# Chthi/Ofighters

Hardware: AMD Instinct MI355X
Metric: arena-steps/sec (env.step+obs+policy fwd) at 4096 arenas, 1/2/4/8 MI355X (higher is better)
Workload: dtype f32; 1 GPU; 4096 arenas x 8 ships per GPU, random-bot actions + step + 2D obs rasterise (u8 maps) + bi-head policy forward for 8 ship(s)/arena, trunk shared per arena (BASELINE configs[3]); arenas_per_gpu=4096, ships=8, laser_cap=512, episode_ticks=200, parallelism=arena-sharded x1, RCCL all-reduce of episodic scores only, laser_overflow=0, last_episode_score_sum=70993, last_episode_arenas=4096

## Files before the change

include/ofx.h:

```cpp
#ifndef OFX_H
#define OFX_H

#include <stddef.h>
#include <stdint.h>

#ifdef __cplusplus
extern "C" {
#endif

#define OFX_VERSION 1

enum {
  OFX_OK = 0,
  OFX_ERR_INVALID = -1,
  OFX_ERR_NO_DEVICE = -2,
  OFX_ERR_HIP = -3,
  OFX_ERR_STATE = -4,
  OFX_ERR_OVERFLOW = -5
};

typedef struct ofx_config {
  int32_t n_arenas;
  int32_t n_ships;
  int32_t laser_cap;
// ... 141 lines not shown
  int32_t n_tensors;
} ofx_policy_desc;
int ofx_policy_layout(const ofx_handle *h, ofx_policy_desc *desc_host);
int ofx_policy_forward(ofx_handle *h, const float *weights, const uint8_t *ship_mask,
                       float *act_values, int32_t *iaction, int32_t *ipointer,
                       float *heatmap);
int ofx_policy_pin_weights(ofx_handle *h, const float *weights);
#define OFX_OPT_TRUNK_PLAIN 1
#define OFX_OPT_FRAMES_REF  2
#define OFX_OPT_TRUNK_FUSE  4
#define OFX_OPT_BILINEAR_LEGACY 3
#define OFX_OPT_POLICY_BF16 5
#define OFX_OPT_FIT_PLAIN 6
#define OFX_OPT_TRUNK_SPARSE 7
int ofx_policy_trunk_stats(ofx_handle *h, int64_t *counts_host);
int ofx_set_option(ofx_handle *h, int32_t option, int32_t value);
int ofx_policy_explore(ofx_handle *h, double epsilon, uint64_t seed, uint32_t tick, int32_t collecting,
                       const uint8_t *ship_mask, int32_t *iaction, int32_t *ipointer);
int ofx_policy_epsilon_ladder(ofx_handle *h, const double *expo_host);
int ofx_policy_epsilon_ladder_host(ofx_handle *h, double *dst_host);
int ofx_policy_act(ofx_handle *h, const float *weights, const uint8_t *ship_mask, double epsilon, uint64_t seed,
                   uint32_t tick, int32_t collecting, float *q_sa, float *p_sp, float *v_act, float *v_ptr);
int ofx_policy_act_boltzmann(ofx_handle *h, const float *weights, const uint8_t *ship_mask, double epsilon,
                             float tau_act, float tau_ptr, uint64_t seed, uint32_t tick, int32_t collecting,
                             float *q_sa, float *p_sp, float *v_act, float *v_ptr);
int ofx_policy_gumbel(ofx_handle *h, const uint32_t *words_dev, int32_t n, float *g_dev);
int ofx_policy_actions(ofx_handle *h, const int32_t *iaction, const int32_t *ipointer,
                       const uint8_t *ship_mask, ofx_action *actions);

typedef struct ofx_transition {
// ... 125 lines not shown
```

ofighters_amd/_native.py:

```python
import ctypes as C
import os

_HERE = os.path.dirname(os.path.abspath(__file__))
LIB_PATH = os.path.join(_HERE, "libofx.so")

OFX_OK = 0
OFX_ERR_INVALID = -1
OFX_ERR_NO_DEVICE = -2
OFX_ERR_HIP = -3
OFX_ERR_STATE = -4
OFX_ERR_OVERFLOW = -5

BOT_IDLE, BOT_RANDOM, BOT_TURRET, BOT_RUNNER, BOT_THRUST, BOT_SHOOT = range(6)
BEHAVIOURS = {None: BOT_IDLE, "idle": BOT_IDLE, "random": BOT_RANDOM, "turret": BOT_TURRET,
              "runner": BOT_RUNNER, "thrust": BOT_THRUST, "shoot": BOT_SHOOT}

(F_SHIP_X, F_SHIP_Y, F_SHIP_PX, F_SHIP_PY, F_SHIP_ALIVE, F_REWARD, F_SCORE, F_N_LASERS, F_LASER_X, F_LASER_Y,
 F_LASER_OWNER, F_LASER_DEAD, F_KILLER, F_TIME, F_LAST_SCORES, F_HULL, F_LASER_DX, F_LASER_DY,
 F_OBS_REWARD) = range(19)

MAP_U8, MAP_F32, MAP_F64, MAP_BITS = range(4)
OPT_TRUNK_PLAIN, OPT_FRAMES_REF, OPT_BILINEAR_LEGACY, OPT_TRUNK_FUSE, OPT_POLICY_BF16, OPT_FIT_PLAIN, OPT_TRUNK_SPARSE = 1, 2, 3, 4, 5, 6, 7


# ... 140 lines not shown
    "ofx_dqn_targets_nstep": (_i, [_vp, _vp, C.c_int32, _vp, _vp, _vp, _vp, _vp, _vp, _vp, _vp, _vp]),
    "ofx_dqn_targets_double": (_i, [_vp, _vp, _vp, C.c_int32, _vp, _vp, _vp, C.c_float, _vp, _vp, _vp, _vp, _vp, _vp]),
    "ofx_policy_blend_weights": (_i, [_vp, _vp, _vp, C.c_float]),
    "ofx_policy_forward_obs_soft": (_i, [_vp, _vp, C.c_int32, _vp, _vp, C.c_float, _vp, _vp, _vp, _vp, _vp, _vp, _vp, _vp, _vp]),
    "ofx_dqn_targets_soft": (_i, [_vp, _vp, C.c_int32, _vp, _vp, _vp, C.c_float, _vp, _vp, C.c_float, C.c_float, C.c_float,
                                  C.c_float, _vp, _vp, _vp, _vp]),
    "ofx_obs_transform": (_i, [_vp, C.c_int32, _vp, _vp, _vp, _vp]),
    "ofx_replay_augment": (_i, [_vp, _u64, _u32, C.c_int32, C.c_int32, _u32, _vp, _vp, _vp, _vp]),
    "ofx_timer_start": (_i, [_vp]),
    "ofx_timer_stop": (_i, [_vp, C.POINTER(C.c_float)]),
    "ofx_event_record": (_i, [_vp, C.c_int32]),
    "ofx_policy_profile": (_i, [_vp, C.c_int32]),
    "ofx_policy_pin_weights": (_i, [_vp, _vp]),
    "ofx_set_option": (_i, [_vp, C.c_int32, C.c_int32]),
    "ofx_policy_trunk_stats": (_i, [_vp, C.POINTER(C.c_int64)]),
    "ofx_event_elapsed": (_i, [_vp, C.c_int32, C.c_int32, C.POINTER(C.c_float)]),
}

_LIB = None


def lib():
    global _LIB
    if _LIB is None:
        if not os.path.exists(LIB_PATH):
            raise ImportError(
                "ofighters_amd: %s is missing - build it with `make -C ofighters_amd/csrc` "
                "(there is no CPU fallback)" % LIB_PATH)
        L = C.CDLL(LIB_PATH)
        for name, (res, args) in SIGNATURES.items():
# ... 21 lines not shown
```

ofighters_amd/csrc/ofx_policy.hip:

```cpp
#include <string.h>

#include "ofx_internal.h"
#include "ofx_arena.h"
#include "ofx_blob.h"
#include "ofx_trunk.h"
#include "ofx_head.h"

typedef float f32x16 __attribute__((ext_vector_type(16)));
typedef float f32x4 __attribute__((ext_vector_type(4)));


extern "C" int ofx_policy_layout(const ofx_handle *h, ofx_policy_desc *desc) {
  (void)h;
  if (!desc) { ofx_set_error("ofx_policy_layout: null desc"); return OFX_ERR_INVALID; }
  memset(desc, 0, sizeof(*desc));
  desc->n_tensors = policy_layout(desc->offset, desc->count);
  desc->n_floats = desc->offset[desc->n_tensors];
  return OFX_OK;
}

struct PrepLayout {
  int tw[4], tb[4];
  int uw[3], ub[3];
  int w3mf;
// ... 574 lines not shown
  const int a = s / M, i = s - a * M;
  const float a0 = act[2 * s], a1 = act[2 * s + 1], T = t_act[s];
  int ia = a1 > a0 ? 1 : 0;
  if (T != 0.f) {
    uint32_t r[4];
    ofx_philox4x32_10((uint32_t)(arena_base + a), (uint32_t)i, tick, OFX_STREAM_BOLTZMANN_ACT, k0, k1, r);
    ia = fmaf(T, hd_gumbel(r[1]), a1) > fmaf(T, hd_gumbel(r[0]), a0) ? 1 : 0;
  }
  iaction[s] = ia;
  q_sa[s] = ia ? a1 : a0;
  v_act[s] = fmaxf(a0, a1);
}

struct PolicyWs {
  float *p1, *p2, *p3, *p4, *g1, *d1, *u0, *up1, *u2fr, *vfr, *c4;
  unsigned long long *best;
  int32_t *iaction, *ipointer, *live;
  float *t_act, *t_ptr, *cand_raw;
  unsigned long long *cand_key;
  unsigned *cand_max;
  float *soft_m, *soft_z;
};

constexpr int kDense1Chunks = 25;

static void policy_layout_ws(Arena &A, bool fused, size_t N, size_t S, bool sample, bool soft, PolicyWs &W) {
  size_t f2, f3, f4;
  ofx_head_frame_bytes(S, &f2, &f3, &f4);
  W.p1 = A.f(fused ? 0 : N * 8 * 200 * 200);
  W.p2 = A.f(N * 8 * 100 * 100); W.p3 = A.f(N * 8 * 50 * 50); W.p4 = A.f(N * 5000); W.g1 = A.f(N * 100 * kDense1Chunks);
  W.d1 = A.f(S * 100); W.u0 = A.f(S * 625); W.up1 = A.f(S * 2 * 50 * 50);
  W.u2fr = (float *)A.take(f2); W.vfr = (float *)A.take(f3); W.c4 = (float *)A.take(f4);
  W.best = A.n<unsigned long long>(S); W.iaction = A.n<int32_t>(S); W.ipointer = A.n<int32_t>(2 * S); W.live = A.n<int32_t>(S + 1);
  const size_t Q = sample ? S : 0;
  W.t_act = A.f(Q); W.t_ptr = A.f(Q); W.cand_raw = A.f(8 * Q); W.cand_key = A.n<unsigned long long>(8 * Q); W.cand_max = A.n<unsigned>(8 * Q);
  const size_t Qs = soft ? S : 0;
  W.soft_m = A.f(8 * Qs); W.soft_z = A.f(8 * Qs);
}
static int policy_workspace(ofx_handle *h, PolicyWs *ws, size_t N, size_t S, bool sample = false, bool soft = false) {
  const bool fused = ofx_trunk_fused(h, N);
  Arena measure;
  policy_layout_ws(measure, fused, N, S, sample, soft, *ws);
  const int rc = ofx_ensure_scratch(h, measure.used);
  if (rc) return rc;
  Arena A(h->scratch, measure.used);
  policy_layout_ws(A, fused, N, S, sample, soft, *ws);
  if (!A.ok()) { ofx_set_error("policy forward: internal workspace sized too small"); return OFX_ERR_STATE; }
  return OFX_OK;
}

int ofx_launch_gemm(ofx_handle *h, const float *A, int lda, const float *B, int ldb, const float *bias, float *C, int ldc,
                    int M, int N, int K, int relu, const int32_t *live) {
  const int tiles_m = (M + 31) / 32, tiles_n = (N + 31) / 32, tiles = tiles_m * tiles_n;
  if (K == 100 && lda % 4 == 0 && ((uintptr_t)A & 15) == 0)
    hipLaunchKernelGGL(k_gemm_f32_k100, dim3((unsigned)(((tiles_m + 3) / 4) * tiles_n)), dim3(256), 0, h->stream, A, lda, B, ldb,
                       bias, C, ldc, M, N, relu, live, tiles_n);
  else
    hipLaunchKernelGGL(k_gemm_f32, dim3((tiles + 3) / 4), dim3(256), 0, h->stream, A, lda, B, ldb, bias, C, ldc, M, N, K,
                       relu, live);
  OFX_HIP(hipGetLastError());
  return OFX_OK;
}

// ... 43 lines not shown
  if (h->prep_pinned && h->prep_pinned == weights) return policy_prepare(h, weights, &h->prep);
  return OFX_OK;
}

extern "C" int ofx_set_option(ofx_handle *h, int32_t option, int32_t value) {
  if (!h) { ofx_set_error("ofx_set_option: null handle"); return OFX_ERR_INVALID; }
  switch (option) {
    case OFX_OPT_TRUNK_PLAIN: h->opt_trunk_plain = value != 0; return OFX_OK;
    case OFX_OPT_TRUNK_FUSE:
      if (value < 0 || value > 2) { ofx_set_error("ofx_set_option: OFX_OPT_TRUNK_FUSE takes 0 (auto), 1 (always), 2 (never)"); return OFX_ERR_INVALID; }
      h->opt_trunk_fuse = value; return OFX_OK;
    case OFX_OPT_FRAMES_REF: h->opt_frames_ref = value != 0; return OFX_OK;
    case OFX_OPT_TRUNK_SPARSE:
      if (value && !h->trunk_stat) {
        OFX_HIP(hipSetDevice(h->cfg.device));
        OFX_HIP(hipMalloc((void **)&h->trunk_stat, 4 * sizeof(unsigned long long)));
        OFX_HIP(hipMemsetAsync(h->trunk_stat, 0, 4 * sizeof(unsigned long long), h->stream));
      }
      h->opt_trunk_dense = value == 0; h->opt_trunk_count = value != 0; return OFX_OK;
    case OFX_OPT_FIT_PLAIN: h->opt_fit_plain = value != 0; return OFX_OK;
    case OFX_OPT_POLICY_BF16:
      if (value < 0 || value > 2) { ofx_set_error("ofx_set_option: OFX_OPT_POLICY_BF16 takes 0 (fp32), 1 (bf16 operands), 2 (fp16 operands)"); return OFX_ERR_INVALID; }
      h->opt_policy_lowp = value; return OFX_OK;
    case OFX_OPT_BILINEAR_LEGACY:
      if (h->opt_bilinear_legacy == (value != 0)) return OFX_OK;
      h->opt_bilinear_legacy = value != 0;
      OFX_HIP(hipSetDevice(h->cfg.device));
      return h->prep_pinned ? policy_prepare(h, h->prep_pinned, &h->prep) : OFX_OK;
    default: ofx_set_error("ofx_set_option: unknown option %d", option); return OFX_ERR_INVALID;
  }
}

// ... 24 lines not shown
  int32_t off[64], cnt[64];
  policy_layout(off, cnt);
  const PrepLayout L = prep_layout();

  const bool pinned = h->prep && h->prep_pinned == weights;
  if (!pinned && (rc = policy_prepare(h, weights, &h->prep_tmp))) return rc;
  const float *prep = pinned ? h->prep : h->prep_tmp;

  const int lowp = a.vec8 == nullptr ? h->opt_policy_lowp : 0;
  TrunkParams tp;
  memset(&tp, 0, sizeof(tp));
  tp.bits[0] = a.bits[0]; tp.bits[1] = a.bits[1]; tp.bits_stride = a.bits_stride; tp.images = N;
  for (int i = 0; i < 4; i++) { tp.tw[i] = prep + L.tw[i]; tp.tb[i] = prep + L.tb[i]; }
  for (int i = 0; i < 3; i++) tp.wbm[i] = prep + L.wbm[i];
  tp.lut1 = prep + L.lut1; tp.zero16 = prep + L.zero16;
  tp.p1 = ws.p1; tp.p2 = ws.p2; tp.p3 = ws.p3; tp.p4 = ws.p4;
  tp.lowp = lowp; tp.sparse = !h->opt_trunk_dense || a.vec8 != nullptr;
  tp.stat = h->opt_trunk_count ? h->trunk_stat : nullptr;
  if ((rc = ofx_launch_trunk(h, tp))) return rc;

  const float *k1 = weights + off[OFX_T_DENSE1];
  {
    static_assert(5000 == kDense1Chunks * kSplitKc, "k_gemm_f32_splitk's chunk");
    const int tiles_n = (100 + 31) / 32, groups_m = ((N + 31) / 32 + 3) / 4;
    hipLaunchKernelGGL(k_gemm_f32_splitk, dim3((unsigned)(tiles_n * groups_m * kDense1Chunks)), dim3(256), 0, h->stream, ws.p4,
                       5000, k1 + 8 * 100, 100, ws.g1, N, 100, tiles_n, groups_m);
    OFX_HIP(hipGetLastError());
  }
  HeadParams hp;
  hp.N = N; hp.M = a.M; hp.st = h->st; hp.vec8 = a.vec8; hp.g1 = ws.g1; hp.g1_chunks = kDense1Chunks;
  hp.k1 = k1; hp.b1 = weights + off[OFX_T_DENSE1 + 1];
// ... 380 lines not shown
```

ofighters_amd/csrc/ofx_trunk.h:

```cpp
#pragma once
#include "ofx_internal.h"

#define PS 400

struct ConvParams {
  const float *in;
  const unsigned *bits[2];
  size_t bits_stride;
  const float *w, *b;
  float *out;
  const uint8_t *mask;
  const float *wbm;
  int H, W;
  int tiles_x, tiles;
  int legacy;
  int images;
  const int32_t *live;
  unsigned long long *stat;
};

struct TrunkParams {
  const unsigned *bits[2];
  size_t bits_stride;
  int images;
  const float *tw[4], *tb[4], *wbm[3], *lut1, *zero16;
  float *p1, *p2, *p3, *p4;
  int lowp;
  bool sparse;
  unsigned long long *stat;
};

bool ofx_trunk_fused(const ofx_handle *h, size_t images);
int ofx_launch_trunk(ofx_handle *h, const TrunkParams &p);
int ofx_launch_conv1_lut(ofx_handle *h, const void *bits, int n, const float *lut, float *out);
```

ofighters_amd/csrc/ofx_trunk.hip:

```cpp
#include "ofx_trunk.h"
#include "ofx_diag.h"
#include "ofx_lowp.h"

typedef float f32x4 __attribute__((ext_vector_type(4)));
typedef float f32x2 __attribute__((ext_vector_type(2)));

template <int CIN, int COUT, int TH, int TW, int MODE, bool POOL, bool OUT_HWC>
__global__ __launch_bounds__(((TH / 2) * (TW / 2) + 63) / 64 * 64) void k_conv(ConvParams p) {
  constexpr int NT = (TH / 2) * (TW / 2);
  constexpr int NTB = (NT + 63) / 64 * 64;
  constexpr int TWP = TW + 2;
  __shared__ __align__(16) float tile[CIN][TH + 2][TWP];
  const int img = blockIdx.x / p.tiles, t = blockIdx.x - img * p.tiles;
  if (p.mask && !p.mask[img]) return;
  const int ty0 = (t / p.tiles_x) * TH, tx0 = (t % p.tiles_x) * TW;
  const int tid = threadIdx.x;
  const int H = p.H, W = p.W;

  constexpr int TOTAL = CIN * (TH + 2) * TWP;
  constexpr int SU = 8;
  for (int base = 0; base < TOTAL; base += NTB * SU) {
    float vals[SU];
#pragma unroll
    for (int u = 0; u < SU; u++) {
// ... 409 lines not shown
      } else {
        f32x4 d0 = binit;
#pragma unroll
        for (int j = 0; j < NK; j++) d0 = __builtin_amdgcn_mfma_f32_16x16x4f32(a0[aof(j)], bw[j], d0, 0, 0, 0);
        finish(d0, T);
      }
    }
  }
}

template <int WD, int RP, int LS, int PLS, int LP>
__device__ __forceinline__ void ts_gemm_phase_sparse(const float *abase, const float (&bw)[LP ? 1 : 24], const lp_x4 (&bwb)[6],
                                                     const f32x4 binit, int wv, int lane,
                                                     int n16, int kq, int r, float *orow, const unsigned *nz, float k2,
                                                     bool top, bool bottom, unsigned &n_exec, unsigned &n_all,
                                                     unsigned long long *dbg = nullptr) {
#if OFX_TRUNK_STAMPS
  unsigned long long g_last = __builtin_amdgcn_s_memtime();
#define TSG_STAMP(i) do { const unsigned long long t_ = __builtin_amdgcn_s_memtime(); dbg[i] += t_ - g_last; g_last = t_; } while (0)
#else
#define TSG_STAMP(i) do { } while (0)
#endif
  constexpr int NK = 24, NPX = RP * WD, NT = (NPX + 15) / 16;
  static_assert(WD % 4 == 0 && NT <= 64, "four M-tiles per wave at most");
  auto aof = [&](int j) -> int { return (4 * (j & 1)) * PLS + ((j >> 1) / 3) * LS + ((j >> 1) % 3); };
  int toff[6];
#pragma unroll
  for (int J = 0; J < 6; J++) {
    const int tap = 2 * J + (kq >> 1);
    toff[J] = (4 * (kq & 1) - kq) * PLS + (tap / 3) * LS + tap % 3;
  }
// ... 31 lines not shown
    float q0, q1;
    q0 = max_raw(max_raw(d[0], 0.f), d[1]);
    q1 = max_raw(max_raw(d[2], 0.f), d[3]);
    q0 = max_raw(q0, __builtin_bit_cast(float, __builtin_amdgcn_mov_dpp(__builtin_bit_cast(int, q0), 0xB1, 0xF, 0xF, true)));
    q1 = max_raw(q1, __builtin_bit_cast(float, __builtin_amdgcn_mov_dpp(__builtin_bit_cast(int, q1), 0xB1, 0xF, 0xF, true)));
    const int P = 16 * T + 4 * kq;
    const int rp = P / WD, x = P - rp * WD;
    if (r == 0 && P < NPX) *reinterpret_cast<float2 *>(orow + rp * (WD / 2) + (x >> 1)) = make_float2(q0, q1);
  };
  auto a_of_tile = [&](int T) -> const float * {
    const int P = min(16 * T + n16, NPX - 1);
    const int rp = P / WD, x = P - rp * WD;
    return abase + 2 * rp * LS + x;
  };
  unsigned long long run_mask;
  {
    const int T = lane, P = 16 * T, rp = P / WD, x = P - rp * WD;
    bool run = T < NT;
    if (run && !(x < 1 || x + 15 > WD - 2 || P + 15 >= NPX || (top && rp == 0) || (bottom && rp == RP - 1))) {
      const int w0 = (x - 1) >> 5, lo = (x - 1) & 31;
      const unsigned m0 = 0x3FFFFu << lo, m1 = lo + 18 > 32 ? (1u << (lo + 18 - 32)) - 1u : 0u;
      unsigned any = 0u;
#pragma unroll
      for (int rr = 0; rr < 4; rr++) {
        const unsigned *rw = nz + (2 * rp + rr) * 8 + w0;
        any |= (rw[0] & m0) | (rw[1] & m1);
      }
      run = any != 0u;
    }
    run_mask = __builtin_amdgcn_ballot_w64(run);
  }
  auto store_const = [&](int T) {
    const int P = 16 * T + 4 * kq, rp = P / WD, x = P - rp * WD;
    if (r == 0) *reinterpret_cast<float2 *>(orow + rp * (WD / 2) + (x >> 1)) = make_float2(k2, k2);
  };
  auto run1 = [&](int T0) {
    f32x4 d0 = binit;
    mm1(a_of_tile(T0), d0);
    finish(d0, T0);
  };
#pragma unroll 1
  for (int T = wv; T < NT; T += 16)
    if (!((run_mask >> T) & 1ull)) store_const(T);
  if (wv == 0) { n_all += (unsigned)NT; n_exec += (unsigned)__builtin_popcountll(run_mask); }
  TSG_STAMP(0);
  unsigned long long m = run_mask;
  for (int i = 0; i < wv && m; i++) m &= m - 1;
#pragma unroll 1
  while (m) {
    const int T0 = __builtin_ctzll(m);
    unsigned long long m2 = m;
    for (int i = 0; i < 16 && m2; i++) m2 &= m2 - 1;
    if (m2) {
      const int T1 = __builtin_ctzll(m2);
      f32x4 d0 = binit, d1 = binit;
      mm2(a_of_tile(T0), a_of_tile(T1), d0, d1);
      finish(d0, T0);
      finish(d1, T1);
      for (int i = 0; i < 16 && m2; i++) m2 &= m2 - 1;
    } else run1(T0);
    m = m2;
  }
  TSG_STAMP(2);
}

template <int WD, int RP, int LS, int PLS, int LP>
__device__ __forceinline__ void ts_gemm_phase_bf16(const float *abase, const lp_x4 (&bwb)[6], const f32x4 binit, int wv, int n16,
                                                   int kq, int r, float *orow) {
  constexpr int NPX = RP * WD, NT = (NPX + 15) / 16;
  static_assert(WD % 4 == 0 && NT <= 64, "four M-tiles per wave at most");
  int toff[6];
#pragma unroll
  for (int J = 0; J < 6; J++) {
    const int tap = 2 * J + (kq >> 1);
    toff[J] = (4 * (kq & 1) - kq) * PLS + (tap / 3) * LS + tap % 3;
  }
// ... 23 lines not shown
      const float *q0 = a0 + toff[J], *q1 = a1 + toff[J];
      const lp_x4 A0 = lp_pk4<LP>(q0[0], q0[PLS], q0[2 * PLS], q0[3 * PLS]);
      const lp_x4 A1 = lp_pk4<LP>(q1[0], q1[PLS], q1[2 * PLS], q1[3 * PLS]);
      d0 = lp_mfma16<LP>(A0, bwb[J], d0);
      d1 = lp_mfma16<LP>(A1, bwb[J], d1);
    }
    finish(d0, T);
    if (two) finish(d1, T1);
  }
}

constexpr int F12_TH = 10, F12_LS = 216, F12_ROWS = F12_TH + 2;
constexpr int F12_PLS = (F12_ROWS * F12_LS + 63) / 64 * 64 + 16;
constexpr int F12_WR = 14, F12_BR = 2 * (F12_TH + 1) + 2;
constexpr int F12_THREADS = 1024;
static_assert(F12_PLS % 64 == 16 && F12_PLS % 4 == 0 && F12_LS % 4 == 0, "tile layout");
static_assert(2 * F12_BR * F12_WR <= F12_THREADS, "one staged word per thread");
static_assert((F12_TH + 1) * 100 <= 2 * F12_THREADS && F12_TH * 100 <= F12_THREADS, "pixel pairs per step");

template <int LP, bool SPARSE = false>
__global__ __launch_bounds__(F12_THREADS) void k_trunk12(ConvParams p, const float *lut) {
  constexpr bool BF16 = LP != 0;
  constexpr int W = PS, H = PS, H1 = PS / 2, H2 = PS / 4, LS = F12_LS, PLS = F12_PLS, NK = 24;
  __shared__ __align__(16) float slut[2 * 512 * 8];
  __shared__ __align__(16) float tile[8 * F12_PLS];
  __shared__ unsigned rows[2][2][F12_BR][F12_WR];
  __shared__ __align__(16) float halo[2][8][2][F12_LS];
  __shared__ unsigned nz[SPARSE ? 2 : 1][F12_ROWS][8];
  __shared__ __align__(16) float k1s[8], k2s[8];
  __shared__ float wbs[(SPARSE && !BF16) ? 24 * 64 : 1];
  unsigned n_exec = 0, n_all = 0, t_exec = 0, t_all = 0;
#if OFX_TRUNK_STAMPS
  unsigned long long st_a = 0, st_b = 0, st_last = __builtin_amdgcn_s_memtime(), st_begin = st_last, st_g[3] = {0, 0, 0};
#define T12_STAMP(acc) do { const unsigned long long t_ = __builtin_amdgcn_s_memtime(); acc += t_ - st_last; st_last = t_; } while (0)
#else
#define T12_STAMP(acc) do { } while (0)
#endif
  const int tid = threadIdx.x, lane = tid & 63;
  const int wv = __builtin_amdgcn_readfirstlane(tid >> 6);
  const int n16 = lane & 15, kq = lane >> 4, co = n16 >> 1, r = n16 & 1;

  auto bits_fetch = [&](int img, int pa, int pb) -> unsigned {
    const int nrows = 2 * (pb - pa) + 2;
    unsigned out = 0u;
// ... 51 lines not shown
      f32x4 d0 = binit;
      if constexpr (BF16) {
#pragma unroll
        for (int J = 0; J < 6; J++) {
          const int tap = 2 * J + (kq >> 1);
          const float *q0 = a0 + (4 * (kq & 1) - kq) * PLS + (tap / 3) * LS + tap % 3;
          d0 = lp_mfma16<LP ? LP : 1>(lp_pk4<LP ? LP : 1>(q0[0], q0[PLS], q0[2 * PLS], q0[3 * PLS]), bwb[J], d0);
        }
      } else {
        auto aof = [&](int j) -> int { return (4 * (j & 1)) * PLS + ((j >> 1) / 3) * LS + ((j >> 1) % 3); };
#pragma unroll
        for (int j = 0; j < NK; j++) d0 = __builtin_amdgcn_mfma_f32_16x16x4f32(a0[aof(j)], wbs[(BF16 ? 0 : j) * 64 + lane], d0, 0, 0, 0);
      }
      float q0 = max_raw(max_raw(d0[0], 0.f), d0[1]);
      q0 = max_raw(q0, __builtin_bit_cast(float, __builtin_amdgcn_mov_dpp(__builtin_bit_cast(int, q0), 0xB1, 0xF, 0xF, true)));
      if (r == 0 && kq == 0) k2s[co] = q0;
    }
    __syncthreads();
    for (int e = tid; e < 8 * PLS / 4; e += F12_THREADS) reinterpret_cast<f32x4 *>(tile)[e] = f32x4{0.f, 0.f, 0.f, 0.f};
  }
  bits_commit(0, 0, F12_TH + 1, bits_fetch((int)blockIdx.x, 0, F12_TH + 1));
  unsigned w_ahead = 0u;
  if constexpr (SPARSE) { if ((int)blockIdx.x < p.images) w_ahead = bits_fetch((int)blockIdx.x, F12_TH + 1, 2 * F12_TH + 1); }
  __syncthreads();
  const float k2 = SPARSE ? k2s[co] : 0.f;

#pragma unroll 1
  for (int img = (int)blockIdx.x; img < p.images; img += (int)gridDim.x)
#pragma unroll 1
  for (int step = 0; step < H1 / F12_TH; step++) {
    const int R0 = step * F12_TH;
// ... 85 lines not shown
      if (++s2 == H1 / F12_TH) { s2 = 0; i2 += (int)gridDim.x; }
      const int r2 = s2 * F12_TH;
      w_ahead = i2 < p.images ? bits_fetch(i2, s2 ? r2 + 1 : 0, min(r2 + F12_TH + 1, H1)) : 0u;
    }

    if constexpr (SPARSE) {
      float bwl[BF16 ? 1 : NK];
      if constexpr (!BF16) {
        int zoff;
        asm volatile("s_mov_b32 %0, 0" : "=s"(zoff));
#pragma unroll
        for (int j = 0; j < NK; j++) bwl[j] = wbs[j * 64 + lane + zoff];
      }
      ts_gemm_phase_sparse<200, F12_TH / 2, F12_LS, F12_PLS, LP>(abase, bwl, bwb, binit, wv, lane, n16, kq, r,
                                                                  p.out + (((size_t)img * 8 + co) * H2 + (R0 >> 1)) * H2,
                                                                  &nz[buf][0][0], k2, step == 0, last, n_exec, n_all
#if OFX_TRUNK_STAMPS
                                                                  , st_g
#endif
                                                                  );
      for (int e = tid; e < F12_ROWS * 8; e += F12_THREADS) (&nz[buf ^ 1][0][0])[e] = 0u;
    } else if constexpr (BF16)
      ts_gemm_phase_bf16<200, F12_TH / 2, F12_LS, F12_PLS, LP ? LP : 1>(abase, bwb, binit, wv, n16, kq, r,
                                                            p.out + (((size_t)img * 8 + co) * H2 + (R0 >> 1)) * H2);
    else
      ts_gemm_phase<200, F12_TH / 2, F12_LS, F12_PLS>(abase, bw, binit, wv, n16, kq, r,
                                                       p.out + (((size_t)img * 8 + co) * H2 + (R0 >> 1)) * H2);
    if constexpr (!SPARSE) { if (more) bits_commit(buf ^ 1, na, nb, nextw); }
    __syncthreads();
  }
  if constexpr (SPARSE) {
#if OFX_TRUNK_STAMPS
    T12_STAMP(st_b);
    if (p.stat && tid == 0) {
      atomicAdd(&p.stat[0], st_a); atomicAdd(&p.stat[1], st_b);
      atomicAdd(&p.stat[2], st_g[0]); atomicAdd(&p.stat[3], st_g[2]);
    }
#else
    if (p.stat && lane == 0) {
      atomicAdd(&p.stat[0], (unsigned long long)n_exec); atomicAdd(&p.stat[1], (unsigned long long)n_all);
      atomicAdd(&p.stat[2], (unsigned long long)t_exec); atomicAdd(&p.stat[3], (unsigned long long)t_all);
    }
#endif
  }
}

constexpr int C3_W = 100, C3_TH = 20, C3_LS = 108, C3_ROWS = C3_TH + 2, C3_F4 = C3_LS / 4;
constexpr int C3_PLS = (C3_ROWS * C3_LS + 63) / 64 * 64 + 16;
constexpr int C3_PF4 = C3_ROWS * C3_F4, C3_NI = (C3_PF4 + 63) / 64;
static_assert(C3_PLS % 64 == 16 && C3_W % C3_TH == 0 && C3_W / 4 + 2 == C3_F4 && 64 * C3_NI * 4 <= C3_PLS + 64 * 4, "tile layout");
static_assert(2 * 8 * C3_PLS * 4 <= 160 * 1024, "two tiles in LDS");

template <int LP>
__global__ __launch_bounds__(F12_THREADS) void k_conv3_stream(ConvParams p, const float *zero16) {
  constexpr bool BF16 = LP != 0;
  constexpr int W = C3_W, H = C3_W, H2 = C3_W / 2, PLS = C3_PLS, NK = 24, STEPS = H / C3_TH;
  __shared__ __align__(16) float tiles[2][8 * C3_PLS];
  const int tid = threadIdx.x, lane = tid & 63;
  const int wv = __builtin_amdgcn_readfirstlane(tid >> 6);
  const int n16 = lane & 15, kq = lane >> 4, co = n16 >> 1, r = n16 & 1;

  auto stage = [&](int buf, int img, int R0) {
#pragma unroll 1
    for (int i = wv; i < 8 * C3_NI; i += F12_THREADS / 64) {
      const int ci = i / C3_NI, k = i - ci * C3_NI;
      const int q = 64 * k + lane;
      if (q < C3_PF4) {
        const int row = q / C3_F4, c4 = q - row * C3_F4, gy = R0 - 1 + row;
        const float *src = zero16;
        if (c4 >= 1 && c4 <= W / 4 && gy >= 0 && gy < H) src = p.in + (((size_t)img * 8 + ci) * H + gy) * W + 4 * (c4 - 1);
        __builtin_amdgcn_global_load_lds((const __attribute__((address_space(1))) void *)src,
                                         (__attribute__((address_space(3))) void *)&tiles[buf][ci * PLS + 256 * k], 16, 0, 0);
      }
    }
  };

  float bw[BF16 ? 1 : NK];
  lp_x4 bwb[6];
  if constexpr (BF16) ts_bw_lp<LP ? LP : 1>(p.wbm, n16, kq, bwb);
  else {
#pragma unroll
    for (int j = 0; j < NK; j++) bw[j] = p.wbm[j * 64 + lane];
  }
  const float bias = p.b[co];
  const f32x4 binit = {bias, bias, bias, bias};
  if ((int)blockIdx.x < p.images) stage(0, (int)blockIdx.x, 0);
  __builtin_amdgcn_s_waitcnt(0x0F70);
  __syncthreads();
  int buf = 0;
#pragma unroll 1
  for (int img = (int)blockIdx.x; img < p.images; img += (int)gridDim.x)
#pragma unroll 1
  for (int step = 0; step < STEPS; step++) {
    const int R0 = step * C3_TH;
    const bool last = step + 1 == STEPS;
    const int nimg = last ? img + (int)gridDim.x : img;
    if (nimg < p.images) stage(buf ^ 1, nimg, last ? 0 : R0 + C3_TH);
    if constexpr (BF16)
      ts_gemm_phase_bf16<W, C3_TH / 2, C3_LS, C3_PLS, LP ? LP : 1>(&tiles[buf][kq * PLS + 3], bwb, binit, wv, n16, kq, r,
                                                      p.out + (((size_t)img * 8 + co) * H2 + (R0 >> 1)) * H2);
    else
      ts_gemm_phase<W, C3_TH / 2, C3_LS, C3_PLS>(&tiles[buf][kq * PLS + 3], bw, binit, wv, n16, kq, r,
                                                 p.out + (((size_t)img * 8 + co) * H2 + (R0 >> 1)) * H2);
    __builtin_amdgcn_s_waitcnt(0x0F70);
    __syncthreads();
    buf ^= 1;
  }
}

bool ofx_trunk_fused(const ofx_handle *h, size_t N) {
  if (h->opt_trunk_plain) return false;
  return h->opt_trunk_fuse == 1 || (h->opt_trunk_fuse == 0 && N >= 4 * (size_t)h->n_cus);
}

template <int CIN, int COUT, int TH, int TW, int MODE, bool POOL, bool OUT_HWC>
static int launch_conv(ofx_handle *h, ConvParams p, int images, int H) {
  p.H = H; p.W = H;
  p.tiles_x = H / TW;
  p.tiles = p.tiles_x * (H / TH);
  constexpr int NTB = ((TH / 2) * (TW / 2) + 63) / 64 * 64;
  hipLaunchKernelGGL((k_conv<CIN, COUT, TH, TW, MODE, POOL, OUT_HWC>), dim3((unsigned)(images * p.tiles)), dim3(NTB), 0,
// ... 15 lines not shown
  cp.bits[1] = cp.bits[0] + (PS * PS) / 32;
  cp.bits_stride = 2 * (size_t)((PS * PS) / 32);
  cp.out = out; cp.images = n;
  return launch_conv1_lut(h, cp, lut);
}

static void trunk_layer(ConvParams &cp, const TrunkParams &p, int i, const float *in, float *out) {
  cp.in = in; cp.w = p.tw[i]; cp.b = p.tb[i]; cp.out = out;
  if (i > 0) cp.wbm = p.wbm[i - 1];
}

template <int LP>
static int trunk_streaming(ofx_handle *h, ConvParams cp, const TrunkParams &p) {
  const dim3 grid((unsigned)(p.images < h->n_cus ? p.images : h->n_cus));
  cp.w = p.tw[0]; cp.b = p.tb[1]; cp.out = p.p2; cp.wbm = p.wbm[0]; cp.stat = p.stat;
  if (p.sparse) hipLaunchKernelGGL((k_trunk12<LP, true>), grid, dim3(F12_THREADS), 0, h->stream, cp, p.lut1);
  else hipLaunchKernelGGL((k_trunk12<LP, false>), grid, dim3(F12_THREADS), 0, h->stream, cp, p.lut1);
  OFX_HIP(hipGetLastError());
  trunk_layer(cp, p, 2, p.p2, p.p3);
  hipLaunchKernelGGL(k_conv3_stream<LP>, grid, dim3(F12_THREADS), 0, h->stream, cp, p.zero16);
  OFX_HIP(hipGetLastError());
  trunk_layer(cp, p, 3, p.p3, p.p4);
  return launch_convm<8, 10, 4, 0, true, 1, LP>(h, cp, p.images, 50);
}

int ofx_launch_trunk(ofx_handle *h, const TrunkParams &p) {
  ConvParams cp{};
  cp.bits[0] = p.bits[0]; cp.bits[1] = p.bits[1]; cp.bits_stride = p.bits_stride; cp.images = p.images;
  const bool plain = h->opt_trunk_plain;
  if (ofx_trunk_fused(h, (size_t)p.images))
    return p.lowp == 1 ? trunk_streaming<1>(h, cp, p) : p.lowp == 2 ? trunk_streaming<2>(h, cp, p) : trunk_streaming<0>(h, cp, p);
  const int N = p.images;
  int rc;
  trunk_layer(cp, p, 0, nullptr, p.p1);
  if ((rc = plain ? launch_conv<2, 8, 10, 100, 1, true, false>(h, cp, N, 400) : launch_conv1_lut(h, cp, p.lut1))) return rc;
// ... 3 lines not shown
  if ((rc = plain ? launch_conv<8, 8, 10, 100, 0, true, false>(h, cp, N, 100) : launch_convm<8, 4, 7, 0, false, 1>(h, cp, N, 100))) return rc;
  trunk_layer(cp, p, 3, p.p3, p.p4);
  return plain ? launch_conv<8, 8, 10, 50, 0, true, true>(h, cp, N, 50) : launch_convm<8, 10, 4, 0, true, 1>(h, cp, N, 50);
}

extern "C" int ofx_policy_trunk_stats(ofx_handle *h, int64_t *counts_host) {
  if (!h || !counts_host) { ofx_set_error("ofx_policy_trunk_stats: null argument"); return OFX_ERR_INVALID; }
  for (int i = 0; i < 4; i++) counts_host[i] = 0;
  if (!h->trunk_stat) return OFX_OK;
  OFX_HIP(hipSetDevice(h->cfg.device));
  OFX_HIP(hipMemcpyAsync(counts_host, h->trunk_stat, 4 * sizeof(unsigned long long), hipMemcpyDeviceToHost, h->stream));
  OFX_HIP(hipMemsetAsync(h->trunk_stat, 0, 4 * sizeof(unsigned long long), h->stream));
  OFX_HIP(hipStreamSynchronize(h->stream));
  return OFX_OK;
}
```

ofighters_amd/engine.py:

```python
import ctypes as C

import numpy as np

from . import _native as nat

_FIELD_DTYPE = {
    nat.F_SHIP_X: np.int32, nat.F_SHIP_Y: np.int32, nat.F_SHIP_PX: np.int32, nat.F_SHIP_PY: np.int32,
    nat.F_SHIP_ALIVE: np.uint8, nat.F_REWARD: np.int32, nat.F_SCORE: np.int32, nat.F_N_LASERS: np.int32,
    nat.F_LASER_X: np.float64, nat.F_LASER_Y: np.float64, nat.F_LASER_OWNER: np.uint8,
    nat.F_LASER_DEAD: np.uint8, nat.F_KILLER: np.int16, nat.F_TIME: np.int32, nat.F_LAST_SCORES: np.int32,
    nat.F_HULL: np.int32, nat.F_LASER_DX: np.float64, nat.F_LASER_DY: np.float64, nat.F_OBS_REWARD: np.int32,
}
_MAP_DTYPE = {nat.MAP_U8: np.uint8, nat.MAP_F32: np.float32, nat.MAP_F64: np.float64, nat.MAP_BITS: np.uint8}

ACTION_DTYPE = np.dtype([("px", np.int32), ("py", np.int32), ("shoot", np.uint8), ("thrust", np.uint8),
                         ("valid", np.uint8), ("_pad", np.uint8)])
assert ACTION_DTYPE.itemsize == C.sizeof(nat.OfxAction) == 12


class DeviceBuffer:

    def __init__(self, nbytes):
        self.nbytes = int(nbytes)
        p = C.c_void_p()
# ... 322 lines not shown
                       heat_ptr=None):
        nat.check(nat.lib().ofx_policy_forward(self._h, weights_ptr, ship_mask_ptr, act_ptr, iaction_ptr,
                                               ipointer_ptr, heat_ptr))

    def policy_pin_weights(self, weights_ptr):
        nat.check(nat.lib().ofx_policy_pin_weights(self._h, weights_ptr))

    def set_option(self, option, value):
        nat.check(nat.lib().ofx_set_option(self._h, int(option), int(value)))

    def policy_trunk_stats(self):
        v = (C.c_int64 * 4)()
        nat.check(nat.lib().ofx_policy_trunk_stats(self._h, v))
        return tuple(int(x) for x in v)

    def policy_actions(self, out_ptr=None, iaction_ptr=None, ipointer_ptr=None, ship_mask_ptr=None):
        out_ptr = out_ptr or self._actions.ptr
        nat.check(nat.lib().ofx_policy_actions(self._h, iaction_ptr, ipointer_ptr, ship_mask_ptr, out_ptr))
        return out_ptr

    def policy_forward_host(self, weights, ship_mask=None, want_heat=False):
        S = self.N * self.M
        w = np.ascontiguousarray(weights, np.float32)
        dw = DeviceBuffer(w.nbytes).upload(w)
        dm = None
        if ship_mask is not None:
            m = np.ascontiguousarray(ship_mask, np.uint8).reshape(S)
            dm = DeviceBuffer(m.nbytes).upload(m)
        da, di, dp = DeviceBuffer(8 * S), DeviceBuffer(4 * S), DeviceBuffer(8 * S)
        dh = DeviceBuffer(4 * S * self.W * self.H) if want_heat else None
# ... 455 lines not shown
```

Measured before the change: 230,600 arena-steps/s.

## Propagate conv2 sparsity marks to skip constant tiles in streaming conv3

The fused conv1/2 kernel now writes per-row bitmasks of non-constant pooled outputs, plus the constant fill value K2, to global buffers. A new sparse variant of the streaming conv3 kernel loads these marks into LDS, precomputes the constant output K3, and runs only the MFMA tiles whose inputs are non-constant. The tile-distribution loop across waves is also replaced with a mbcnt/ballot rank, removing serial bit-popping. This adds mark stores and loads and a small one-time K3 computation per block, plus stats and debug entry points.

New measurement: 233,900 arena-steps/s, median of 6. 1.01x the previous value.

```diff
diff --git a/include/ofx.h b/include/ofx.h
--- a/include/ofx.h
+++ b/include/ofx.h
@@ -179,6 +179,8 @@
 #define OFX_OPT_FIT_PLAIN 6
 #define OFX_OPT_TRUNK_SPARSE 7
 int ofx_policy_trunk_stats(ofx_handle *h, int64_t *counts_host);
+int ofx_policy_trunk_stats3(ofx_handle *h, int64_t *run_host, int64_t *total_host);
+int ofx_policy_trunk_features(ofx_handle *h, int32_t n_images, int32_t m, float *out_host);
 int ofx_set_option(ofx_handle *h, int32_t option, int32_t value);
 int ofx_policy_explore(ofx_handle *h, double epsilon, uint64_t seed, uint32_t tick, int32_t collecting,
                        const uint8_t *ship_mask, int32_t *iaction, int32_t *ipointer);
diff --git a/ofighters_amd/_native.py b/ofighters_amd/_native.py
--- a/ofighters_amd/_native.py
+++ b/ofighters_amd/_native.py
@@ -178,6 +178,8 @@
     "ofx_policy_pin_weights": (_i, [_vp, _vp]),
     "ofx_set_option": (_i, [_vp, C.c_int32, C.c_int32]),
     "ofx_policy_trunk_stats": (_i, [_vp, C.POINTER(C.c_int64)]),
+    "ofx_policy_trunk_stats3": (_i, [_vp, C.POINTER(C.c_int64), C.POINTER(C.c_int64)]),
+    "ofx_policy_trunk_features": (_i, [_vp, C.c_int32, C.c_int32, _vp]),
     "ofx_event_elapsed": (_i, [_vp, C.c_int32, C.c_int32, C.POINTER(C.c_float)]),
 }
 
diff --git a/ofighters_amd/csrc/ofx_policy.hip b/ofighters_amd/csrc/ofx_policy.hip
--- a/ofighters_amd/csrc/ofx_policy.hip
+++ b/ofighters_amd/csrc/ofx_policy.hip
@@ -612,6 +612,8 @@
 
 struct PolicyWs {
   float *p1, *p2, *p3, *p4, *g1, *d1, *u0, *up1, *u2fr, *vfr, *c4;
+  unsigned *nz2;
+  float *k2;
   unsigned long long *best;
   int32_t *iaction, *ipointer, *live;
   float *t_act, *t_ptr, *cand_raw;
@@ -629,6 +631,7 @@
   W.p2 = A.f(N * 8 * 100 * 100); W.p3 = A.f(N * 8 * 50 * 50); W.p4 = A.f(N * 5000); W.g1 = A.f(N * 100 * kDense1Chunks);
   W.d1 = A.f(S * 100); W.u0 = A.f(S * 625); W.up1 = A.f(S * 2 * 50 * 50);
   W.u2fr = (float *)A.take(f2); W.vfr = (float *)A.take(f3); W.c4 = (float *)A.take(f4);
+  W.nz2 = A.n<unsigned>(fused ? N * 100 * 4 : 0); W.k2 = A.f(fused ? 8 : 0);
   W.best = A.n<unsigned long long>(S); W.iaction = A.n<int32_t>(S); W.ipointer = A.n<int32_t>(2 * S); W.live = A.n<int32_t>(S + 1);
   const size_t Q = sample ? S : 0;
   W.t_act = A.f(Q); W.t_ptr = A.f(Q); W.cand_raw = A.f(8 * Q); W.cand_key = A.n<unsigned long long>(8 * Q); W.cand_max = A.n<unsigned>(8 * Q);
@@ -645,6 +648,16 @@
   policy_layout_ws(A, fused, N, S, sample, soft, *ws);
   if (!A.ok()) { ofx_set_error("policy forward: internal workspace sized too small"); return OFX_ERR_STATE; }
   return OFX_OK;
+}
+
+const float *ofx_policy_ws_p4(ofx_handle *h, size_t N, size_t S) {
+  PolicyWs ws;
+  Arena measure;
+  policy_layout_ws(measure, ofx_trunk_fused(h, N), N, S, false, false, ws);
+  if (!h->scratch || h->scratch_bytes < measure.used) return nullptr;
+  Arena A(h->scratch, measure.used);
+  policy_layout_ws(A, ofx_trunk_fused(h, N), N, S, false, false, ws);
+  return A.ok() ? ws.p4 : nullptr;
 }
 
 int ofx_launch_gemm(ofx_handle *h, const float *A, int lda, const float *B, int ldb, const float *bias, float *C, int ldc,
@@ -718,8 +731,8 @@
     case OFX_OPT_TRUNK_SPARSE:
       if (value && !h->trunk_stat) {
         OFX_HIP(hipSetDevice(h->cfg.device));
-        OFX_HIP(hipMalloc((void **)&h->trunk_stat, 4 * sizeof(unsigned long long)));
-        OFX_HIP(hipMemsetAsync(h->trunk_stat, 0, 4 * sizeof(unsigned long long), h->stream));
+        OFX_HIP(hipMalloc((void **)&h->trunk_stat, 6 * sizeof(unsigned long long)));
+        OFX_HIP(hipMemsetAsync(h->trunk_stat, 0, 6 * sizeof(unsigned long long), h->stream));
       }
       h->opt_trunk_dense = value == 0; h->opt_trunk_count = value != 0; return OFX_OK;
     case OFX_OPT_FIT_PLAIN: h->opt_fit_plain = value != 0; return OFX_OK;
@@ -774,7 +787,7 @@
   for (int i = 0; i < 4; i++) { tp.tw[i] = prep + L.tw[i]; tp.tb[i] = prep + L.tb[i]; }
   for (int i = 0; i < 3; i++) tp.wbm[i] = prep + L.wbm[i];
   tp.lut1 = prep + L.lut1; tp.zero16 = prep + L.zero16;
-  tp.p1 = ws.p1; tp.p2 = ws.p2; tp.p3 = ws.p3; tp.p4 = ws.p4;
+  tp.p1 = ws.p1; tp.p2 = ws.p2; tp.p3 = ws.p3; tp.p4 = ws.p4; tp.nz2 = ws.nz2; tp.k2 = ws.k2;
   tp.lowp = lowp; tp.sparse = !h->opt_trunk_dense || a.vec8 != nullptr;
   tp.stat = h->opt_trunk_count ? h->trunk_stat : nullptr;
   if ((rc = ofx_launch_trunk(h, tp))) return rc;
diff --git a/ofighters_amd/csrc/ofx_trunk.h b/ofighters_amd/csrc/ofx_trunk.h
--- a/ofighters_amd/csrc/ofx_trunk.h
+++ b/ofighters_amd/csrc/ofx_trunk.h
@@ -17,6 +17,8 @@
   int images;
   const int32_t *live;
   unsigned long long *stat;
+  unsigned *marks;
+  float *k2;
 };
 
 struct TrunkParams {
@@ -28,8 +30,11 @@
   int lowp;
   bool sparse;
   unsigned long long *stat;
+  unsigned *nz2;
+  float *k2;
 };
 
 bool ofx_trunk_fused(const ofx_handle *h, size_t images);
 int ofx_launch_trunk(ofx_handle *h, const TrunkParams &p);
+const float *ofx_policy_ws_p4(ofx_handle *h, size_t N, size_t S);
 int ofx_launch_conv1_lut(ofx_handle *h, const void *bits, int n, const float *lut, float *out);
diff --git a/ofighters_amd/csrc/ofx_trunk.hip b/ofighters_amd/csrc/ofx_trunk.hip
--- a/ofighters_amd/csrc/ofx_trunk.hip
+++ b/ofighters_amd/csrc/ofx_trunk.hip
@@ -447,7 +447,7 @@
                                                      const f32x4 binit, int wv, int lane,
                                                      int n16, int kq, int r, float *orow, const unsigned *nz, float k2,
                                                      bool top, bool bottom, unsigned &n_exec, unsigned &n_all,
-                                                     unsigned long long *dbg = nullptr) {
+                                                     unsigned *marks = nullptr, unsigned long long *dbg = nullptr) {
 #if OFX_TRUNK_STAMPS
   unsigned long long g_last = __builtin_amdgcn_s_memtime();
 #define TSG_STAMP(i) do { const unsigned long long t_ = __builtin_amdgcn_s_memtime(); dbg[i] += t_ - g_last; g_last = t_; } while (0)
@@ -509,9 +509,10 @@
     return abase + 2 * rp * LS + x;
   };
   unsigned long long run_mask;
+  bool run;
   {
     const int T = lane, P = 16 * T, rp = P / WD, x = P - rp * WD;
-    bool run = T < NT;
+    run = T < NT;
     if (run && !(x < 1 || x + 15 > WD - 2 || P + 15 >= NPX || (top && rp == 0) || (bottom && rp == RP - 1))) {
       const int w0 = (x - 1) >> 5, lo = (x - 1) & 31;
       const unsigned m0 = 0x3FFFFu << lo, m1 = lo + 18 > 32 ? (1u << (lo + 18 - 32)) - 1u : 0u;
@@ -524,6 +525,20 @@
       run = any != 0u;
     }
     run_mask = __builtin_amdgcn_ballot_w64(run);
+  }
+  if (marks != nullptr && wv == 15) {
+    constexpr int W2 = WD / 2, WPR = (W2 + 31) / 32;
+    static_assert(RP * WPR <= 64, "one lane per word");
+    if (lane < RP * WPR) {
+      const int y = lane / WPR, w = lane - y * WPR;
+      const int f0 = y * W2 + 32 * w, t0 = f0 >> 3;
+      const unsigned b5 = (unsigned)(run_mask >> t0);
+      const unsigned lo = (((b5 & 15u) * 0x00204081u) & 0x01010101u) * 0xFFu, hi = ((b5 >> 4) & 1u) * 0xFFu;
+      unsigned word = __funnelshift_r(lo, hi, (unsigned)(f0 & 7));
+      const int nb = W2 - 32 * w;
+      if (nb < 32) word &= (1u << nb) - 1u;
+      marks[lane] = word;
+    }
   }
   auto store_const = [&](int T) {
     const int P = 16 * T + 4 * kq, rp = P / WD, x = P - rp * WD;
@@ -539,22 +554,20 @@
     if (!((run_mask >> T) & 1ull)) store_const(T);
   if (wv == 0) { n_all += (unsigned)NT; n_exec += (unsigned)__builtin_popcountll(run_mask); }
   TSG_STAMP(0);
-  unsigned long long m = run_mask;
-  for (int i = 0; i < wv && m; i++) m &= m - 1;
+  const unsigned rank = __builtin_amdgcn_mbcnt_hi((unsigned)(run_mask >> 32), __builtin_amdgcn_mbcnt_lo((unsigned)run_mask, 0u));
+  unsigned long long m = __builtin_amdgcn_ballot_w64(run && (rank & 15u) == (unsigned)wv);
 #pragma unroll 1
   while (m) {
     const int T0 = __builtin_ctzll(m);
-    unsigned long long m2 = m;
-    for (int i = 0; i < 16 && m2; i++) m2 &= m2 - 1;
-    if (m2) {
-      const int T1 = __builtin_ctzll(m2);
+    m &= m - 1;
+    if (m) {
+      const int T1 = __builtin_ctzll(m);
+      m &= m - 1;
       f32x4 d0 = binit, d1 = binit;
       mm2(a_of_tile(T0), a_of_tile(T1), d0, d1);
       finish(d0, T0);
       finish(d1, T1);
-      for (int i = 0; i < 16 && m2; i++) m2 &= m2 - 1;
     } else run1(T0);
-    m = m2;
   }
   TSG_STAMP(2);
 }
@@ -608,6 +621,7 @@
 constexpr int F12_PLS = (F12_ROWS * F12_LS + 63) / 64 * 64 + 16;
 constexpr int F12_WR = 14, F12_BR = 2 * (F12_TH + 1) + 2;
 constexpr int F12_THREADS = 1024;
+constexpr int C3_MW = 4;
 static_assert(F12_PLS % 64 == 16 && F12_PLS % 4 == 0 && F12_LS % 4 == 0, "tile layout");
 static_assert(2 * F12_BR * F12_WR <= F12_THREADS, "one staged word per thread");
 static_assert((F12_TH + 1) * 100 <= 2 * F12_THREADS && F12_TH * 100 <= F12_THREADS, "pixel pairs per step");
@@ -622,6 +636,7 @@
   __shared__ __align__(16) float halo[2][8][2][F12_LS];
   __shared__ unsigned nz[SPARSE ? 2 : 1][F12_ROWS][8];
   __shared__ __align__(16) float k1s[8], k2s[8];
+  __shared__ unsigned mk2[SPARSE ? (F12_TH / 2) * C3_MW : 1];
   __shared__ float wbs[(SPARSE && !BF16) ? 24 * 64 : 1];
   unsigned n_exec = 0, n_all = 0, t_exec = 0, t_all = 0;
 #if OFX_TRUNK_STAMPS
@@ -703,7 +718,10 @@
       }
       float q0 = max_raw(max_raw(d0[0], 0.f), d0[1]);
       q0 = max_raw(q0, __builtin_bit_cast(float, __builtin_amdgcn_mov_dpp(__builtin_bit_cast(int, q0), 0xB1, 0xF, 0xF, true)));
-      if (r == 0 && kq == 0) k2s[co] = q0;
+      if (r == 0 && kq == 0) {
+        k2s[co] = q0;
+        if (blockIdx.x == 0 && p.k2) p.k2[co] = q0;
+      }
     }
     __syncthreads();
     for (int e = tid; e < 8 * PLS / 4; e += F12_THREADS) reinterpret_cast<f32x4 *>(tile)[e] = f32x4{0.f, 0.f, 0.f, 0.f};
@@ -819,7 +837,7 @@
       }
       ts_gemm_phase_sparse<200, F12_TH / 2, F12_LS, F12_PLS, LP>(abase, bwl, bwb, binit, wv, lane, n16, kq, r,
                                                                   p.out + (((size_t)img * 8 + co) * H2 + (R0 >> 1)) * H2,
-                                                                  &nz[buf][0][0], k2, step == 0, last, n_exec, n_all
+                                                                  &nz[buf][0][0], k2, step == 0, last, n_exec, n_all, mk2
 #if OFX_TRUNK_STAMPS
                                                                   , st_g
 #endif
@@ -833,6 +851,7 @@
                                                        p.out + (((size_t)img * 8 + co) * H2 + (R0 >> 1)) * H2);
     if constexpr (!SPARSE) { if (more) bits_commit(buf ^ 1, na, nb, nextw); }
     __syncthreads();
+    if constexpr (SPARSE) { if (tid < (F12_TH / 2) * C3_MW) p.marks[((size_t)img * H2 + (R0 >> 1)) * C3_MW + tid] = mk2[tid]; }
   }
   if constexpr (SPARSE) {
 #if OFX_TRUNK_STAMPS
@@ -856,11 +875,15 @@
 static_assert(C3_PLS % 64 == 16 && C3_W % C3_TH == 0 && C3_W / 4 + 2 == C3_F4 && 64 * C3_NI * 4 <= C3_PLS + 64 * 4, "tile layout");
 static_assert(2 * 8 * C3_PLS * 4 <= 160 * 1024, "two tiles in LDS");
 
-template <int LP>
+template <int LP, bool SPARSE = false>
 __global__ __launch_bounds__(F12_THREADS) void k_conv3_stream(ConvParams p, const float *zero16) {
   constexpr bool BF16 = LP != 0;
   constexpr int W = C3_W, H = C3_W, H2 = C3_W / 2, PLS = C3_PLS, NK = 24, STEPS = H / C3_TH;
   __shared__ __align__(16) float tiles[2][8 * C3_PLS];
+  __shared__ __align__(16) unsigned nzs[SPARSE ? 2 : 1][SPARSE ? C3_ROWS : 1][8];
+  __shared__ float k3s[8];
+  static_assert((2 * 8 * C3_PLS + 2 * C3_ROWS * 8 + 8) * 4 <= 160 * 1024, "tiles, marks and K3 in LDS");
+  unsigned n_exec = 0, n_all = 0;
   const int tid = threadIdx.x, lane = tid & 63;
   const int wv = __builtin_amdgcn_readfirstlane(tid >> 6);
   const int n16 = lane & 15, kq = lane >> 4, co = n16 >> 1, r = n16 & 1;
@@ -878,6 +901,18 @@
                                          (__attribute__((address_space(3))) void *)&tiles[buf][ci * PLS + 256 * k], 16, 0, 0);
       }
     }
+    if constexpr (SPARSE) {
+      constexpr int NM = (C3_ROWS * 8 + 63) / 64;
+      const int k = F12_THREADS / 64 - 1 - wv;
+      const int q = 64 * k + lane;
+      if (k < NM && q < C3_ROWS * 8) {
+        const int row = q >> 3, w = q & 7, gy = R0 - 1 + row;
+        const unsigned *src = reinterpret_cast<const unsigned *>(zero16);
+        if (w < C3_MW && gy >= 0 && gy < H) src = p.marks + ((size_t)img * H + gy) * C3_MW + w;
+        __builtin_amdgcn_global_load_lds((const __attribute__((address_space(1))) void *)src,
+                                         (__attribute__((address_space(3))) void *)(&nzs[buf][0][0] + 64 * k), 4, 0, 0);
+      }
+    }
   };
 
   float bw[BF16 ? 1 : NK];
@@ -890,8 +925,32 @@
   const float bias = p.b[co];
   const f32x4 binit = {bias, bias, bias, bias};
   if ((int)blockIdx.x < p.images) stage(0, (int)blockIdx.x, 0);
+  if constexpr (SPARSE) {
+    for (int e = tid; e < 8 * 4 * C3_LS; e += F12_THREADS) tiles[1][(e / (4 * C3_LS)) * PLS + e % (4 * C3_LS)] = p.k2[e / (4 * C3_LS)];
+    __syncthreads();
+    if (wv == 0) {
+      const float *a0 = &tiles[1][kq * PLS + 3] + 16 + n16;
+      f32x4 d0 = binit;
+      if constexpr (BF16) {
+#pragma unroll
+        for (int J = 0; J < 6; J++) {
+          const int tap = 2 * J + (kq >> 1);
+          const float *q0 = a0 + (4 * (kq & 1) - kq) * PLS + (tap / 3) * C3_LS + tap % 3;
+          d0 = lp_mfma16<LP ? LP : 1>(lp_pk4<LP ? LP : 1>(q0[0], q0[PLS], q0[2 * PLS], q0[3 * PLS]), bwb[J], d0);
+        }
+      } else {
+        auto aof = [&](int j) -> int { return (4 * (j & 1)) * PLS + ((j >> 1) / 3) * C3_LS + ((j >> 1) % 3); };
+#pragma unroll
+        for (int j = 0; j < NK; j++) d0 = __builtin_amdgcn_mfma_f32_16x16x4f32(a0[aof(j)], bw[BF16 ? 0 : j], d0, 0, 0, 0);
+      }
+      float q0 = max_raw(max_raw(d0[0], 0.f), d0[1]);
+      q0 = max_raw(q0, __builtin_bit_cast(float, __builtin_amdgcn_mov_dpp(__builtin_bit_cast(int, q0), 0xB1, 0xF, 0xF, true)));
+      if (r == 0 && kq == 0) k3s[co] = q0;
+    }
+  }
   __builtin_amdgcn_s_waitcnt(0x0F70);
   __syncthreads();
+  const float k3 = SPARSE ? k3s[co] : 0.f;
   int buf = 0;
 #pragma unroll 1
   for (int img = (int)blockIdx.x; img < p.images; img += (int)gridDim.x)
@@ -901,7 +960,18 @@
     const bool last = step + 1 == STEPS;
     const int nimg = last ? img + (int)gridDim.x : img;
     if (nimg < p.images) stage(buf ^ 1, nimg, last ? 0 : R0 + C3_TH);
-    if constexpr (BF16)
+    if constexpr (SPARSE) {
+#if OFX_TRUNK_STAMPS
+      unsigned long long st_g[3] = {0, 0, 0};
+#endif
+      ts_gemm_phase_sparse<W, C3_TH / 2, C3_LS, C3_PLS, LP>(&tiles[buf][kq * PLS + 3], bw, bwb, binit, wv, lane, n16, kq, r,
+                                                            p.out + (((size_t)img * 8 + co) * H2 + (R0 >> 1)) * H2,
+                                                            &nzs[buf][0][0], k3, step == 0, last, n_exec, n_all, nullptr
+#if OFX_TRUNK_STAMPS
+                                                            , st_g
+#endif
+                                                            );
+    } else if constexpr (BF16)
       ts_gemm_phase_bf16<W, C3_TH / 2, C3_LS, C3_PLS, LP ? LP : 1>(&tiles[buf][kq * PLS + 3], bwb, binit, wv, n16, kq, r,
                                                       p.out + (((size_t)img * 8 + co) * H2 + (R0 >> 1)) * H2);
     else
@@ -910,6 +980,11 @@
     __builtin_amdgcn_s_waitcnt(0x0F70);
     __syncthreads();
     buf ^= 1;
+  }
+  if constexpr (SPARSE) {
+#if !OFX_TRUNK_STAMPS
+    if (p.stat && tid == 0) { atomicAdd(&p.stat[4], (unsigned long long)n_exec); atomicAdd(&p.stat[5], (unsigned long long)n_all); }
+#endif
   }
 }
 
@@ -955,11 +1030,14 @@
 static int trunk_streaming(ofx_handle *h, ConvParams cp, const TrunkParams &p) {
   const dim3 grid((unsigned)(p.images < h->n_cus ? p.images : h->n_cus));
   cp.w = p.tw[0]; cp.b = p.tb[1]; cp.out = p.p2; cp.wbm = p.wbm[0]; cp.stat = p.stat;
+  if (p.sparse && !(p.nz2 && p.k2)) { ofx_set_error("trunk_streaming: the sparse form needs the marks buffer"); return OFX_ERR_STATE; }
+  cp.marks = p.nz2; cp.k2 = p.k2;
   if (p.sparse) hipLaunchKernelGGL((k_trunk12<LP, true>), grid, dim3(F12_THREADS), 0, h->stream, cp, p.lut1);
   else hipLaunchKernelGGL((k_trunk12<LP, false>), grid, dim3(F12_THREADS), 0, h->stream, cp, p.lut1);
   OFX_HIP(hipGetLastError());
   trunk_layer(cp, p, 2, p.p2, p.p3);
-  hipLaunchKernelGGL(k_conv3_stream<LP>, grid, dim3(F12_THREADS), 0, h->stream, cp, p.zero16);
+  if (p.sparse) hipLaunchKernelGGL((k_conv3_stream<LP, true>), grid, dim3(F12_THREADS), 0, h->stream, cp, p.zero16);
+  else hipLaunchKernelGGL((k_conv3_stream<LP, false>), grid, dim3(F12_THREADS), 0, h->stream, cp, p.zero16);
   OFX_HIP(hipGetLastError());
   trunk_layer(cp, p, 3, p.p3, p.p4);
   return launch_convm<8, 10, 4, 0, true, 1, LP>(h, cp, p.images, 50);
@@ -993,3 +1071,26 @@
   OFX_HIP(hipStreamSynchronize(h->stream));
   return OFX_OK;
 }
+
+extern "C" int ofx_policy_trunk_stats3(ofx_handle *h, int64_t *run_host, int64_t *total_host) {
+  if (!h || !run_host || !total_host) { ofx_set_error("ofx_policy_trunk_stats3: null argument"); return OFX_ERR_INVALID; }
+  *run_host = *total_host = 0;
+  if (!h->trunk_stat) return OFX_OK;
+  unsigned long long v[2] = {0, 0};
+  OFX_HIP(hipSetDevice(h->cfg.device));
+  OFX_HIP(hipMemcpyAsync(v, h->trunk_stat + 4, sizeof(v), hipMemcpyDeviceToHost, h->stream));
+  OFX_HIP(hipMemsetAsync(h->trunk_stat + 4, 0, sizeof(v), h->stream));
+  OFX_HIP(hipStreamSynchronize(h->stream));
+  *run_host = (int64_t)v[0]; *total_host = (int64_t)v[1];
+  return OFX_OK;
+}
+
+extern "C" int ofx_policy_trunk_features(ofx_handle *h, int32_t n_images, int32_t m, float *out_host) {
+  if (!h || !out_host || n_images <= 0 || m <= 0) { ofx_set_error("ofx_policy_trunk_features: bad argument"); return OFX_ERR_INVALID; }
+  const float *p4 = ofx_policy_ws_p4(h, (size_t)n_images, (size_t)n_images * (size_t)m);
+  if (!p4) { ofx_set_error("ofx_policy_trunk_features: no forward of these sizes has run"); return OFX_ERR_STATE; }
+  OFX_HIP(hipSetDevice(h->cfg.device));
+  OFX_HIP(hipMemcpyAsync(out_host, p4, (size_t)n_images * 5000 * sizeof(float), hipMemcpyDeviceToHost, h->stream));
+  OFX_HIP(hipStreamSynchronize(h->stream));
+  return OFX_OK;
+}
diff --git a/ofighters_amd/engine.py b/ofighters_amd/engine.py
--- a/ofighters_amd/engine.py
+++ b/ofighters_amd/engine.py
@@ -360,6 +360,17 @@
         nat.check(nat.lib().ofx_policy_trunk_stats(self._h, v))
         return tuple(int(x) for x in v)
 
+    def policy_trunk_stats3(self):
+        run, total = C.c_int64(), C.c_int64()
+        nat.check(nat.lib().ofx_policy_trunk_stats3(self._h, C.byref(run), C.byref(total)))
+        return int(run.value), int(total.value)
+
+    def policy_trunk_features(self):
+        out = np.empty((self.N, 25, 25, 8), np.float32)
+        self.sync()
+        nat.check(nat.lib().ofx_policy_trunk_features(self._h, self.N, self.M, out.ctypes.data_as(C.c_void_p)))
+        return out
+
     def policy_actions(self, out_ptr=None, iaction_ptr=None, ipointer_ptr=None, ship_mask_ptr=None):
         out_ptr = out_ptr or self._actions.ptr
         nat.check(nat.lib().ofx_policy_actions(self._h, iaction_ptr, ipointer_ptr, ship_mask_ptr, out_ptr))
```
